# hlesmqh/WS3D

Measured on AMD Instinct MI355X. Metric: KITTI scenes/sec (16384 pts) Stage-1 RPN fwd, 1/2/4/8 GPU; FPS+group HBM GB/s, higher is better.
Workload: dtype f32

## Files before the change

include/ws3d_ops.h:

```cpp
#ifndef WS3D_OPS_H
#define WS3D_OPS_H

#include <stddef.h>
#include <stdint.h>

#ifdef __cplusplus
extern "C" {
#endif

#define WS3D_OK 0
#define WS3D_E_INVALID (-1)
#define WS3D_E_LAUNCH (-2)
#define WS3D_E_WORKSPACE (-3)
#define WS3D_E_UNSUPPORTED (-4)

#if defined(__GNUC__)
#define WS3D_API __attribute__((visibility("default")))
#else
#define WS3D_API
#endif

typedef void *ws3d_stream_t;

#define WS3D_ABI_VERSION 6
// ... 97 lines not shown
WS3D_API int ws3d_pgather_gemm2_compact(int b, int n, int m, long max_rows, int o1, int o2, const float *pmat, int p_stride, const float *xyz,
                               const float *new_xyz, const int32_t *rowc, const int32_t *rowsrc, const int32_t *total, const float *w1x,
                               const float *b1, int relu1, const float *w2t, const float *b2, int relu2, float *out, long limit, ws3d_stream_t stream);
WS3D_API int ws3d_pgather_gemm3_compact(int b, int n, int m, long max_rows, int o1, int o2, int o3, const float *pmat, int p_stride, const float *xyz,
                               const float *new_xyz, const int32_t *rowc, const int32_t *rowsrc, const int32_t *total, const float *w1x,
                               const float *b1, int relu1, const float *w2t, const float *b2, int relu2, const float *w3t, const float *b3,
                               float *out, int out_stride, long limit, ws3d_stream_t stream);
WS3D_API int ws3d_gemm_pool_compact(long max_rows, int k_dim, int o_dim, const float *x_rows, const int32_t *rowc, const int32_t *total,
                           const float *wt, const float *bias, float *out, int out_stride, long limit, ws3d_stream_t stream);
typedef struct ws3d_compact_mlp_args {
    int b, n, m;
    long max_rows;
    int o1, o2, o3;
    const float *pmat;
    int p_stride;
    const float *xyz, *new_xyz;
    const int32_t *rowc, *rowsrc, *total;
    const float *w1x, *b1;
    int relu1;
    const float *w2t, *b2;
    int relu2;
    const float *w3t, *b3;
    float *mid;
    float *out;
    int out_stride;
    long limit;
} ws3d_compact_mlp_args;
WS3D_API int ws3d_compact_mlp_pair(int kind, const ws3d_compact_mlp_args *scale0, const ws3d_compact_mlp_args *scale1, ws3d_stream_t stream);
WS3D_API int ws3d_chain_mlp3_ticket_ints(void);
WS3D_API size_t ws3d_chain_mlp3_blob_floats(int o2);
WS3D_API int ws3d_chain_mlp3_pack(const ws3d_compact_mlp_args *scale, float *blob, ws3d_stream_t stream);
WS3D_API int ws3d_chain_mlp3(const ws3d_compact_mlp_args *scale0, const ws3d_compact_mlp_args *scale1, const float *blob0, const float *blob1,
                             int32_t *ticket, int workgroups, ws3d_stream_t stream);

WS3D_API int ws3d_sa_mlp3_pool_compact(int b, int n, int m, long max_rows, int c1, int c2, int c3, const float *xyz, const float *new_xyz,
                              const float *feat, const int32_t *rowc, const int32_t *rowsrc, const int32_t *total, const float *w1t,
                              const float *b1, const float *w2t, const float *b2, const float *w3t, const float *b3, float *out,
                              int out_stride, long limit, ws3d_stream_t stream);

WS3D_API int ws3d_sa_mlp3_pool_lists(int b, int n, int m, int nsample, int c1, int c2, int c3, const float *xyz, const float *new_xyz,
                            const float *feat, const int32_t *nbr, const float *w1t, const float *b1, const float *w2t, const float *b2,
                            const float *w3t, const float *b3, int relu3, float *out, int out_stride, const int32_t *gate, long gate_limit,
                            ws3d_stream_t stream);

WS3D_API int ws3d_interp_gemm(int b, int n, int m, int c2, int c1, int o_dim, const float *known_feats, const float *unknown_feats,
                     const int32_t *idx, const float *weight, const float *wt, const float *bias, int relu, float *out,
                     ws3d_stream_t stream);

WS3D_API size_t ws3d_conv1x1_wgrad_workspace_bytes(int b, int o, int c, long l);
WS3D_API int ws3d_conv1x1_wgrad(int b, int o, int c, long l, const float *grad_out, const float *x, float *grad_w,
                                void *workspace, size_t workspace_bytes, ws3d_stream_t stream);

WS3D_API size_t ws3d_bn_workspace_bytes(int b, int c, long l);
WS3D_API int ws3d_bn_relu_train_fwd(int b, int c, long l, const float *x, const float *gamma, const float *beta, float eps,
                                    float momentum, int relu, float *running_mean, float *running_var,
                                    int64_t *num_batches_tracked, float *y, float *save_mean, float *save_invstd,
                                    void *workspace, size_t workspace_bytes, ws3d_stream_t stream);
WS3D_API int ws3d_bn_relu_train_bwd(int b, int c, long l, const float *x, const float *dy, const float *gamma,
                                    const float *beta, const float *save_mean, const float *save_invstd, int relu, float *dx,
                                    float *dgamma, float *dbeta, void *workspace, size_t workspace_bytes, ws3d_stream_t stream);

WS3D_API int ws3d_three_interpolate(int b, int c, int m, int n, const float *points, const int32_t *idx,
                           const float *weight, float *out, ws3d_stream_t stream);

WS3D_API int ws3d_three_interpolate_grad(int b, int c, int n, int m, const float *grad_out,
                                const int32_t *idx, const float *weight, float *grad_points,
// ... 188 lines not shown
```

ws3d_amd/_lib.py:

```python
from __future__ import annotations

import ctypes as C
import os

_HERE = os.path.dirname(os.path.abspath(__file__))
DIST_MODE = int(os.environ.get("WS3D_DIST_MODE", "0") or 0)
LIB_PATH = os.environ.get("WS3D_HIP_LIB") or os.path.join(
    _HERE, "libws3d_hip.so" if DIST_MODE == 0 else "libws3d_hip_dm%d.so" % DIST_MODE)

E_INVALID, E_LAUNCH, E_WORKSPACE, E_UNSUPPORTED = -1, -2, -3, -4
ABI_VERSION = 6

_vp = C.c_void_p
_i = C.c_int
_f = C.c_float
_sz = C.c_size_t

class CompactMlpArgs(C.Structure):
    _fields_ = [("b", _i), ("n", _i), ("m", _i), ("max_rows", C.c_long), ("o1", _i), ("o2", _i), ("o3", _i), ("pmat", _vp), ("p_stride", _i),
                ("xyz", _vp), ("new_xyz", _vp), ("rowc", _vp), ("rowsrc", _vp), ("total", _vp), ("w1x", _vp), ("b1", _vp), ("relu1", _i),
                ("w2t", _vp), ("b2", _vp), ("relu2", _i), ("w3t", _vp), ("b3", _vp), ("mid", _vp), ("out", _vp), ("out_stride", _i), ("limit", C.c_long)]


SIGNATURES = {
# ... 53 lines not shown
    "ws3d_topk_sorted_ws": (_i, [_i, _i, _i, _vp, _vp, _vp, _vp, C.c_size_t, _vp]),
    "ws3d_topk_sorted_sigmoid": (_i, [_i, _i, _i, _vp, _vp, _vp, _vp]),
    "ws3d_topk_sorted_sigmoid_ws": (_i, [_i, _i, _i, _vp, _vp, _vp, _vp, C.c_size_t, _vp]),
    "ws3d_three_nn_weights": (_i, [C.c_long, _vp, _vp, _vp]),
    "ws3d_three_nn_w": (_i, [_i, _i, _i, _vp, _vp, _vp, _vp, _vp, _vp, _vp]),
    "ws3d_three_nn_wq": (_i, [_i, _i, _i, _vp, _vp, _vp, _vp, _vp, _vp, _vp, _vp]),
    "ws3d_three_nn_jobs": (_i, [_i, _i, _vp, _vp, _vp, _vp, _vp, _vp, _vp, _vp, _vp]),
    "ws3d_bias_act_inplace": (_i, [_i, _i, C.c_long, _i, _vp, _vp, _vp]),
    "ws3d_rowmax_bias_act": (_i, [_i, _i, C.c_long, _i, _i, _vp, _vp, _vp, _vp]),
    "ws3d_boxes_overlap_bev": (_i, [_i, _vp, _i, _vp, _vp, _vp]),
    "ws3d_boxes_iou_bev": (_i, [_i, _vp, _i, _vp, _vp, _vp]),
    "ws3d_boxes_iou3d_paired": (_i, [_i, _vp, _vp, _vp, _vp, _vp, _vp]),
    "ws3d_nms_mask": (_i, [_i, _vp, _f, _i, _i, _vp, _vp]),
    "ws3d_nms_workspace_bytes": (_sz, [_i]),
    "ws3d_nms": (_i, [_i, _vp, _f, _i, _i, _vp, _sz, _vp, _vp, _vp]),
    "ws3d_nms_batched": (_i, [_i, _i, _vp, _f, _i, _i, _vp, _sz, _vp, _vp, _vp]),
    "ws3d_radius_nms_batched": (_i, [_i, _i, _vp, _f, _i, _vp, _sz, _vp, _vp, _vp]),
    "ws3d_gather_gemm": (_i, [_i, _i, _i, _i, _i, _i, _vp, _vp, _vp, _vp, _vp, _vp, _i, _vp, _vp]),
    "ws3d_gather_gemm2": (_i, [_i, _i, _i, _i, _i, _i, _i, _vp, _vp, _vp, _vp, _vp, _vp, _i, _vp, _vp, _i, _vp, _vp]),
    "ws3d_pgather_gemm2": (_i, [_i, _i, _i, _i, _i, _i, _vp, _i, _vp, _vp, _vp, _vp, _vp, _i, _vp, _vp, _i, _vp, _vp, C.c_long, _vp]),
    "ws3d_pgather_rows": (_i, [_i, _i, _i, _i, _i, _vp, _i, _vp, _vp, _vp, _vp, _vp, _i, _vp, _vp]),
    "ws3d_qinterp_rows": (_i, [_i, _i, _i, _i, _vp, _vp, _vp, _vp, _vp, _i, _vp, _vp, _i, _vp, _vp]),
    "ws3d_compact_pairs": (_i, [C.c_long, _i, _vp, _vp, _vp, _vp, _vp]),
    "ws3d_compact_pairs_count": (_i, [C.c_long, _i, _vp, _vp, _vp]),
    "ws3d_compact_pairs_rows": (_i, [C.c_long, _i, _vp, _vp, _vp, _vp, _vp, _vp, _vp]),
    "ws3d_pgather_gemm2_compact": (_i, [_i, _i, _i, C.c_long, _i, _i, _vp, _i, _vp, _vp, _vp, _vp, _vp, _vp, _vp, _i, _vp, _vp, _i, _vp, C.c_long, _vp]),
    "ws3d_pgather_gemm3_compact": (_i, [_i, _i, _i, C.c_long, _i, _i, _i, _vp, _i, _vp, _vp, _vp, _vp, _vp, _vp, _vp, _i, _vp, _vp, _i, _vp, _vp, _vp, _i, C.c_long, _vp]),
    "ws3d_gemm_pool_compact": (_i, [C.c_long, _i, _i, _vp, _vp, _vp, _vp, _vp, _vp, _i, C.c_long, _vp]),
    "ws3d_compact_mlp_pair": (_i, [_i, C.POINTER(CompactMlpArgs), C.POINTER(CompactMlpArgs), _vp]),
    "ws3d_chain_mlp3_ticket_ints": (_i, []),
    "ws3d_chain_mlp3_blob_floats": (_sz, [_i]),
    "ws3d_chain_mlp3_pack": (_i, [C.POINTER(CompactMlpArgs), _vp, _vp]),
    "ws3d_chain_mlp3": (_i, [C.POINTER(CompactMlpArgs), C.POINTER(CompactMlpArgs), _vp, _vp, _vp, _i, _vp]),
    "ws3d_sa_mlp3_pool_compact": (_i, [_i, _i, _i, C.c_long, _i, _i, _i, _vp, _vp, _vp, _vp, _vp, _vp, _vp, _vp, _vp, _vp, _vp, _vp, _vp, _i, C.c_long, _vp]),
    "ws3d_sa_mlp3_pool_lists": (_i, [_i, _i, _i, _i, _i, _i, _i, _vp, _vp, _vp, _vp, _vp, _vp, _vp, _vp, _vp, _vp, _i, _vp, _i, _vp, C.c_long, _vp]),
    "ws3d_interp_gemm": (_i, [_i, _i, _i, _i, _i, _i, _vp, _vp, _vp, _vp, _vp, _vp, _i, _vp, _vp]),
    "ws3d_gather_boxes_bev": (_i, [_i, _i, _i, _vp, _vp, _vp, _vp, _vp]),
    "ws3d_select_proposals": (_i, [_i, _i, _i, _i, _vp, _vp, _vp, _vp, _f, _vp, _vp, _vp, _vp, _vp]),
    "ws3d_decode_gather_boxes_bev": (_i, [_i, _i, _i, _i, _f, _f, _f, _f, _f, _vp, _vp, _vp, _vp, _vp, _vp]),
    "ws3d_select_proposals_packed": (_i, [_i, _i, _i, _i, _vp, _vp, _vp, _vp, _f, _vp, _vp, _vp, _vp, _vp, _vp]),
    "ws3d_select_proposals_send": (_i, [_i, _i, _i, _i, _vp, _vp, _vp, _vp, _f, _vp, _vp, _vp, _vp, _vp, C.c_long, _vp]),
    "ws3d_split_points_clear": (_i, [C.c_long, _i, _vp, _vp, _vp, _vp, C.c_size_t, _vp]),
    "ws3d_roipool3d": (_i, [_i, _i, _i, _i, _i, _vp, _vp, _vp, _vp, _vp, _vp, _vp]),
    "ws3d_roipool3d_fill": (_i, [_i, _i, _i, _i, _i, _vp, _vp, _vp, _vp, _vp, _vp, _vp]),
    "ws3d_roipool3d_workspace_bytes": (C.c_size_t, [_i, _i]),
    "ws3d_roipool3d_ws": (_i, [_i, _i, _i, _i, _i, _vp, _vp, _vp, _vp, _vp, _vp, _i, _vp, C.c_size_t, _vp]),
    "ws3d_pts_in_boxes3d": (_i, [_i, _i, _vp, _vp, _vp, _vp]),
    "ws3d_instance_clouds": (_i, [_i, _i, _i, _i, _i, _f, _i, _f, _vp, _vp, _vp, _vp, _vp, _vp, _vp, _vp, _vp, _vp]),
    "ws3d_instance_clouds_count": (_i, [_i, _i, _i, _f, _vp, _vp, _vp, _vp, _vp]),
    "ws3d_instance_clouds_emit": (_i, [_i, _i, _i, _i, _f, _i, _f, _vp, _vp, _vp, _vp, _vp, _vp, _vp, _vp, _vp, _vp]),
    "ws3d_click_prepare": (_i, [_i, _i, _i, _i, _vp, _f, _f, _f, _f, _vp, _vp, _vp, _vp, _vp, _vp, _vp]),
    "ws3d_kitti_overlaps": (_i, [_i, _i, _i, C.c_long, _vp, _vp, _vp, _vp, _vp, _vp, _vp]),
    "ws3d_kitti_collect_scores": (_i, [_i, _i, _vp, _vp, _vp, _vp, _vp, _vp, _vp, C.c_double, _vp, _vp, _vp]),
    "ws3d_kitti_count_workspace_bytes": (_sz, [_i, _i]),
    "ws3d_kitti_count": (_i, [_i, _i, _i, _i, _vp, _vp, _vp, _vp, _vp, _vp, _vp, _vp, _vp, _vp, _vp, _vp, _vp, C.c_double, _i, _vp,
                              _sz, _vp, _vp]),
    "ws3d_stage2_embed": (_i, [C.c_long, _i, _vp, _vp, _f] + [_vp] * 10 + [_vp, _vp, _vp]),
    "ws3d_stage2_boxes": (_i, [_i, _i, _i, _f, _f, _f, _f, _vp, _vp, _vp, _vp]),
    "ws3d_stage2_select": (_i, [_i, _i, _f, _f, C.POINTER(_f), _f, _vp, _vp, _vp, _vp, _vp, _vp, _vp, _vp, _vp, _vp]),
    "ws3d_stage2_rcnn_loss": (_i, [_i, _i, _i, _f, _f, _f, _f] + [_vp] * 9 + [_vp]),
    "ws3d_stage2_ioun_loss": (_i, [_i] + [_vp] * 10 + [_vp]),
    "ws3d_rpn_center_labels": (_i, [_i, _i, _i, _i, _f, _f, C.c_double] + [_vp] * 5 + [_vp]),
    "ws3d_rpn_loss_workspace_bytes": (_sz, [_i]),
    "ws3d_rpn_loss": (_i, [_i, _i] + [C.c_double] * 6 + [_vp] * 8 + [_vp, _sz, _vp]),
}

# ... 39 lines not shown
```

ws3d_amd/build.py:

```python
from __future__ import annotations

import argparse
import concurrent.futures as cf
import glob
import os
import shutil
import subprocess
import sys

HERE = os.path.dirname(os.path.abspath(__file__))
CSRC = os.path.join(HERE, "csrc")
OBJ = os.path.join(CSRC, "build")
LIB = os.path.join(HERE, "libws3d_hip.so")
DIST_MODES = (0, 1, 2)


def lib_path(dist_mode: int = 0) -> str:
    return LIB if dist_mode == 0 else os.path.join(HERE, "libws3d_hip_dm%d.so" % dist_mode)
ARCH = "gfx950"
SOURCES = ["core.hip", "fps.hip", "fps_v3.hip", "fps_bucket.hip", "fps_nested.hip", "ballquery_group.hip", "interpolate.hip", "roipool3d.hip", "iou3d.hip", "proposals.hip", "scatter_det.hip", "sa_mlp.hip", "bn_relu.hip", "gemm_pool.hip", "conv_wgrad.hip", "chain_mlp.hip", "rpn_heads.hip", "gemm_rows.hip", "kitti_eval.hip", "instance_clouds.hip", "click.hip", "stage2.hip", "stage2_loss.hip", "rpn_targets.hip"]
CXXFLAGS = ["-O3", "-std=c++17", "-fPIC", "-ffp-contract=off", "-fno-fast-math",
            "-fvisibility=hidden", "-Wall", "-Wno-unused-function"]


def hipcc() -> str:
    for cand in (os.environ.get("HIPCC"), shutil.which("hipcc"), "/opt/rocm/bin/hipcc"):
        if cand and os.path.exists(cand):
            return cand
    raise RuntimeError("hipcc not found (looked at $HIPCC, PATH, /opt/rocm/bin)")


def _deps(src: str):
    return [src, *glob.glob(os.path.join(CSRC, "*.h")), os.path.join(HERE, "..", "include", "ws3d_ops.h"),
            os.path.join(CSRC, "exports.map"), os.path.abspath(__file__)]


def _compile(src: str, force: bool, verbose: bool, dist_mode: int = 0) -> str:
    path = os.path.join(CSRC, src)
    obj = os.path.join(OBJ if dist_mode == 0 else OBJ + "_dm%d" % dist_mode, os.path.splitext(src)[0] + ".o")
    if not force and os.path.exists(obj) and all(
            os.path.getmtime(obj) >= os.path.getmtime(d) for d in _deps(path)):
        return obj
    cmd = [hipcc(), f"--offload-arch={ARCH}", *CXXFLAGS, f"-DWS3D_DIST_MODE={dist_mode}", *os.environ.get("WS3D_EXTRA_DEFS", "").split(), "-c", path, "-o", obj]
    if verbose:
        print(" ".join(cmd), flush=True)
    r = subprocess.run(cmd, capture_output=True, text=True)
    if r.returncode != 0:
        raise RuntimeError(f"hipcc failed for {src}:\n{r.stdout}\n{r.stderr}")
    if verbose and r.stderr.strip():
        print(r.stderr)
    return obj


# ... 43 lines not shown
```

ws3d_amd/compat.py:

```python
from __future__ import annotations

import sys
import types

import os

import torch

from . import _lib
from ._lib import Ws3dError, check


def _dev(*tensors):
    dev = None
    for t in tensors:
        if t is None:
            continue
        if not t.is_cuda:
            raise Ws3dError("ws3d_amd ops need HIP ('cuda') tensors; there is no CPU fallback")
        if not t.is_contiguous():
            raise Ws3dError("ws3d_amd ops need contiguous tensors (the reference asserts the same)")
        if dev is None:
            dev = t.device
        elif t.device != dev:
# ... 578 lines not shown
    O2, O3 = w2t.size(1), w3t.size(1)
    rows = rowc.numel()
    lds = 4 * ((o1 + (O2 + 15) // 16 * 16) * 65 + 2 * 16 * 64)
    if (o1 not in (64, 128) or O2 % 4 or O3 % 128 or lds > min(max_lds, 160 * 1024 - 1024) or pmat.dim() != 2 or pmat.size(0) != B * N or pmat.stride(1) != 1 or
            col0 < 0 or col0 + o1 > pmat.size(1) or tuple(w1x.shape) != (3, o1) or w2t.size(0) != o1 or w3t.size(0) != O2 or not w1x.is_contiguous() or
            not w2t.is_contiguous() or not w3t.is_contiguous() or out2d.dim() != 2 or out2d.stride(1) != 1 or col_offset < 0 or col_offset + O3 > out2d.size(1)):
        return False
    with _on(dev):
        check(_lib.load().ws3d_pgather_gemm3_compact(B, N, M, rows, o1, O2, O3, pmat.data_ptr() + 4 * col0, pmat.stride(0), _p(xyz), _p(new_xyz), _p(rowc),
                                                     _p(rowsrc), _p(total), _p(w1x), _p(b1), int(bool(relu1)), _p(w2t), _p(b2), int(bool(relu2)), _p(w3t), _p(b3),
                                                     out2d.data_ptr() + 4 * col_offset, out2d.stride(0), int(limit), _stream()), "pgather_gemm3_compact")
    return True


def gemm_pool_compact(x_rows, pairs, wt, bias, out2d, col_offset, limit=-1):
    rowc, rowsrc, total = pairs
    dev = _dev(x_rows, rowc, wt, out2d)
    _f32(x_rows, "x_rows"); _f32(wt, "wt"); _f32(out2d, "out2d")
    rows, k = x_rows.shape
    o = wt.size(1)
    if (k % 4 or o % 64 or wt.size(0) != k or rows != rowc.numel() or not x_rows.is_contiguous() or not wt.is_contiguous() or out2d.dim() != 2 or
            out2d.stride(1) != 1 or col_offset < 0 or col_offset + o > out2d.size(1)):
        return False
    with _on(dev):
        check(_lib.load().ws3d_gemm_pool_compact(rows, k, o, _p(x_rows), _p(rowc), _p(total), _p(wt), _p(bias), out2d.data_ptr() + 4 * col_offset,
                                                 out2d.stride(0), int(limit), _stream()), "gemm_pool_compact")
    return True


def compact_mlp_pair(kind, scales, max_lds=160 * 1024, mids=None):
    import ctypes as C
    if len(scales) != 2 or scales[0]["o1"] != scales[1]["o1"]:
        return None if kind == 2 else False
    blocks, keep, outs = [], [], []
    for si, a in enumerate(scales):
        rowc, rowsrc, total = a["pairs"]
        pmat, xyz, new_xyz, w1x, w2t, w3t, out2d, o1, col0, col = a["pmat"], a["xyz"], a["new_xyz"], a["w1x"], a["w2t"], a["w3t"], a["out2d"], a["o1"], a["col0"], a["col_offset"]
        dev = _dev(pmat, xyz, new_xyz, rowc, w1x, w2t, w3t, out2d)
        for t_, nm in ((pmat, "pmat"), (xyz, "xyz"), (new_xyz, "new_xyz"), (w1x, "w1x"), (w2t, "w2t"), (w3t, "w3t"), (out2d, "out2d")):
            _f32(t_, nm)
        B, N, M = xyz.size(0), xyz.size(1), new_xyz.size(1)
        O2, O3 = w2t.size(1), w3t.size(1)
        rows = rowc.numel()
        lds3 = 4 * ((o1 + (O2 + 15) // 16 * 16) * 65 + 2 * 16 * 64)
        ok = (O2 % 4 == 0 and pmat.dim() == 2 and pmat.size(0) == B * N and pmat.stride(1) == 1 and col0 >= 0 and col0 + o1 <= pmat.size(1) and
              tuple(w1x.shape) == (3, o1) and w2t.size(0) == o1 and w3t.size(0) == O2 and w1x.is_contiguous() and w2t.is_contiguous() and w3t.is_contiguous() and
              out2d.dim() == 2 and out2d.stride(1) == 1 and col >= 0 and col + O3 <= out2d.size(1))
        if kind == 3:
            ok = ok and o1 in (64, 128) and O3 % 128 == 0 and lds3 <= min(max_lds, 160 * 1024 - 1024)
        elif kind == 2:
            ok = ok and o1 in (64, 128, 256)
        else:
            ok = ok and O3 % 64 == 0 and mids is not None and tuple(mids[si].shape) == (rows, O2) and mids[si].is_contiguous()
        if not ok:
            return None if kind == 2 else False
        mid = mids[si] if kind == 1 else (torch.empty((rows, O2), dtype=torch.float32, device=dev) if kind == 2 else None)
        outs.append(mid)
        keep.append((pmat, xyz, new_xyz, rowc, rowsrc, total, w1x, w2t, w3t, out2d, mid, a["b1"], a["b2"], a["b3"]))
        blocks.append(_lib.CompactMlpArgs(B, N, M, rows, o1, O2, O3, pmat.data_ptr() + 4 * col0, pmat.stride(0), _p(xyz), _p(new_xyz), _p(rowc), _p(rowsrc),
                                          _p(total), _p(w1x), _p(a["b1"]), int(bool(a["relu1"])), _p(w2t), _p(a["b2"]), int(bool(a["relu2"])), _p(w3t), _p(a["b3"]),
                                          _p(mid), out2d.data_ptr() + 4 * col, out2d.stride(0), -1))
    with _on(dev):
        rc = _lib.load().ws3d_compact_mlp_pair(int(kind), C.byref(blocks[0]), C.byref(blocks[1]), _stream())
    if rc == _lib.E_UNSUPPORTED:
        return None if kind == 2 else False
    check(rc, "compact_mlp_pair")
    return outs if kind == 2 else True


CHAIN_WORKGROUPS = 0
TUNE_KEYS = {"chain_wgs": 0, "mlp2_wgs": 1, "sa1_wgs": 2, "fp_wgs": 3, "pair_wgs": 4, "bq_wide_nw": 5}


def tune(name: str, value: int = -1) -> int:
    rc = _lib.load().ws3d_tune(TUNE_KEYS[name], int(value))
    if rc < 0:
        check(rc, "tune")
    return rc


_CHAIN_BLOBS = {}


def chain_ticket_ints() -> int:
    return int(_lib.load().ws3d_chain_mlp3_ticket_ints())


def _chain_blob(block, tensors, dev):
    import ctypes as C
    key = tuple((t.data_ptr(), t._version) if t is not None else None for t in tensors)
    hit = _CHAIN_BLOBS.get(key)
    if hit is None:
        n = int(_lib.load().ws3d_chain_mlp3_blob_floats(block.o2))
        blob = torch.empty(n, dtype=torch.float32, device=dev)
        with _on(dev):
            check(_lib.load().ws3d_chain_mlp3_pack(C.byref(block), _p(blob), _stream()), "chain_mlp3_pack")
        if torch.cuda.is_current_stream_capturing():
            return blob
        hit = _CHAIN_BLOBS[key] = (blob, tensors)
    return hit[0]


def chain_mlp3(scales, ticket):
    import ctypes as C
# ... 890 lines not shown
```

ws3d_amd/csrc/common.h:

```cpp
#pragma once
#include <hip/hip_runtime.h>
#include <stdint.h>

#include "../../include/ws3d_ops.h"

#define WS3D_WAVE 64

namespace ws3d {

void set_error(const char *fmt, ...);
int check_launch(const char *what);
int raise_lds_cap(const void *fn, size_t bytes, const char *what);
int cu_count();

typedef float floatx16 __attribute__((ext_vector_type(16)));

enum : int { TUNE_CHAIN_WGS = 0, TUNE_MLP2_WGS = 1, TUNE_SA1_WGS = 2, TUNE_FP_WGS = 3, TUNE_PAIR_WGS = 4, TUNE_COUNT = 8 };
extern int g_tune[TUNE_COUNT];

static inline hipStream_t as_stream(ws3d_stream_t s) { return reinterpret_cast<hipStream_t>(s); }

#ifndef WS3D_DIST_MODE
#define WS3D_DIST_MODE 0
#endif
__device__ __forceinline__ float sqdist3(float dx, float dy, float dz) {
#if WS3D_DIST_MODE == 0
    return __builtin_fmaf(dz, dz, __builtin_fmaf(dx, dx, dy * dy));
#elif WS3D_DIST_MODE == 1
    return (dx * dx + dy * dy) + dz * dz;
#else
    return __builtin_fmaf(dz, dz, __builtin_fmaf(dy, dy, dx * dx));
#endif
}

__device__ __forceinline__ float cosf_cr(float a) { return (float)cos((double)a); }
__device__ __forceinline__ float sinf_cr(float a) { return (float)sin((double)a); }
__device__ __forceinline__ float atan2f_cr(float y, float x) { return (float)atan2((double)y, (double)x); }

template <int CTRL>
__device__ __forceinline__ float dpp_f(float v) {
    return __builtin_bit_cast(
        float, __builtin_amdgcn_update_dpp(0, __builtin_bit_cast(int, v), CTRL, 0xF, 0xF, false));
}
enum : int {
    DPP_QUAD_XOR1 = 0xB1,
    DPP_QUAD_XOR2 = 0x4E,
    DPP_ROW_HALF_MIRROR = 0x141,
    DPP_ROW_MIRROR = 0x140,
};

// ... 69 lines not shown
```

ws3d_amd/fastpath.py:

```python
from __future__ import annotations

import contextlib
import contextvars

import torch
import torch.nn as nn

from . import compat as _C
from . import nn_blocks, pn2_ops

FUSED_SA_MLP = True
SA1_FROM_LISTS = True
FUSED_GEMM_POOL = True
FUSED_INTERP_GEMM = True
NESTED_FPS = True
GEOMETRY_AHEAD = True
_AHEAD_OVERRIDE = contextvars.ContextVar("ws3d_geometry_ahead", default=None)


@contextlib.contextmanager
def geometry_ahead(on: bool):
    token = _AHEAD_OVERRIDE.set(bool(on))
    try:
        yield
# ... 2 lines not shown


@contextlib.contextmanager
def compact_only_scales(keys):
    token = _COMPACT_ONLY.set(frozenset(keys))
    try:
        yield
    finally:
        _COMPACT_ONLY.reset(token)


def primed_compact_scales(net, pointcloud: torch.Tensor, margin: float = None):
    margin = PRIMED_MARGIN if margin is None else margin
    keys, per_level = set(), {}
    for row in list_fill(net, pointcloud):
        si = per_level.get(row["level"], 0)
        per_level[row["level"]] = si + 1
        if row["fill"] <= margin * COMPACT_MAX_FILL:
            keys.add((row["level"] - 1, si))
    return frozenset(keys)


def _geometry_ahead_now() -> bool:
    v = _AHEAD_OVERRIDE.get()
    return GEOMETRY_AHEAD if v is None else v
GEOMETRY_IN_CAPTURE = False
PER_POINT_L1 = True
COMPACT_MAX_FILL = 0.55
COMPACT_PAIRS = True
PAIR_DISPATCH = "device"
PRIMED_MARGIN = 0.85
_COMPACT_ONLY = contextvars.ContextVar("ws3d_compact_only_scales", default=frozenset())
CHAIN_MLP = True
PAIRED_SCALES = True
MERGED_THREE_NN = True
FUSED_PROLOGUE = True
MERGED_BINNING = True
PER_POINT_FP = True
FUSED_MLP2_ROWS = True
FUSED_HEADS = True
SPLIT_GEMMS = True
FUSED_GATHER_GEMM2 = True
BIN_INPUT_AHEAD = True
FUSED_QINTERP_GEMM_MIN_ROWS = 30000
FUSED_COMPACT3_MAX_LDS = 64 * 1024
FUSED_GATHER_GEMM = True
GRID_MIN_N = 256
DUAL_SCALE_SEARCH = True
NESTED_CHAIN = True
QUERY_CELL_ORDER = True
PARALLEL_SCALES = True
PARALLEL_HEADS = True


def _row_weights(block):
    w, shift, act = block._folded()
    if act is not None and not isinstance(act, nn.ReLU):
        raise NotImplementedError("fast path supports ReLU / no activation only")
    cache = block.__dict__.get("_row_cache")
    if cache is None or cache[0] is not w:
        cache = (w, w.t().contiguous())
        if not torch.cuda.is_current_stream_capturing():
            block.__dict__["_row_cache"] = cache
    return cache[1], shift, act is not None


def _row_weights_xyz_last(block):
    wt, bias, relu = _row_weights(block)
    cache = block.__dict__.get("_row_cache_xyz_last")
    if cache is None or cache[0] is not wt:
        cache = (wt, torch.cat((wt[3:], wt[:3]), dim=0).contiguous())
        if not torch.cuda.is_current_stream_capturing():
            block.__dict__["_row_cache_xyz_last"] = cache
    return cache[1], bias, relu


def _split_rows(block, wt: torch.Tensor, c2: int):
    cache = block.__dict__.get("_split_cache")
    if cache is None or cache[0] is not wt or cache[1] != c2:
        cache = (wt, c2, wt[:c2].contiguous(), wt[c2:].contiguous())
        if not torch.cuda.is_current_stream_capturing():
            block.__dict__["_split_cache"] = cache
    return cache[2], cache[3]


_SPLIT_GEMM_LIBRARY_WINS = frozenset({(512, 1024, 512)})


def _split_gemm_wins(rows: int, k: int, n: int) -> bool:
    return (rows, k, n) not in _SPLIT_GEMM_LIBRARY_WINS


def _split_gemm(x2d: torch.Tensor, holder, key: str, wt: torch.Tensor, bias=None, relu: bool = False):
    if not SPLIT_GEMMS or x2d.dim() != 2 or not _split_gemm_wins(x2d.size(0), wt.size(0), wt.size(1)):
        return None
    packs = holder.__dict__.get("_gemm_rows_packs")
    ent = None if packs is None else packs.get(key)
    if ent is None or ent[0] is not wt:
        if torch.cuda.is_current_stream_capturing():
            return None
        ent = (wt, _C.gemm_rows_pack(wt))
        holder.__dict__.setdefault("_gemm_rows_packs", {})[key] = ent
    if ent[1] is None:
        return None
    return _C.gemm_rows_split(x2d, ent[1], wt.size(1), bias, relu)


def gemm_rows_packs(model):
    return [ent[1] for m in model.modules() for ent in m.__dict__.get("_gemm_rows_packs", {}).values() if ent[1] is not None]


def _layer(x2d: torch.Tensor, block) -> torch.Tensor:
    wt, bias, relu = _row_weights(block)
    y = _split_gemm(x2d, block, "row", wt, bias, relu)
    if y is not None:
        return y
# ... 387 lines not shown
        rows = g.view(-1, g.size(3))
        if not (FUSED_SA_MLP and rows.size(1) == 4 and len(blocks) == 3 and
                _C.sa_mlp3_pool(rows, grouper.nsample, [_row_weights(b) for b in blocks], out, col)):
            y = rows
            for blk in blocks[:-1]:
                y = _layer(y, blk)
            wt, bias, relu = _row_weights(blocks[-1])
            if not (FUSED_GEMM_POOL and _C.gemm_pool(y, wt, bias, relu, grouper.nsample, out, col)):
                _C.rowmax_rows(_layer(y, blocks[-1]), grouper.nsample, out, col)

    def run_paired() -> bool:
        if not (PAIRED_SCALES and COMPACT_PAIRS and PER_POINT_L1 and len(widths) == 2 and all(isinstance(n_, _PairList) for n_ in nbrs)):
            return False
        blk = [_blocks(m_) for m_ in sa.mlps]
        if any(len(b_) != 3 or b_[0].conv.out_channels > 256 for b_ in blk) or blk[0][0].conv.out_channels != blk[1][0].conv.out_channels:
            return False
        if any(_pair_limit(n_.nbr.numel(), True, (level, si_)) != -1 for si_, n_ in enumerate(nbrs)):
            return False
        if pp[0] is None:
            pp[0] = _per_point_l1(sa, feats, nbrs)
        pmat, offs, w1xs = pp[0]
        scales = []
        for si_ in range(2):
            _w1, b1, r1 = _row_weights_xyz_last(blk[si_][0])
            wt2, b2, r2 = _row_weights(blk[si_][1])
            wt3, b3, r3 = _row_weights(blk[si_][2])
            if not r3:
                return False
            scales.append({"pmat": pmat, "col0": offs[si_], "o1": blk[si_][0].conv.out_channels, "xyz": xyz, "new_xyz": new_xyz, "pairs": nbrs[si_].pairs,
                           "w1x": w1xs[si_], "b1": b1, "relu1": r1, "w2t": wt2, "b2": b2, "relu2": r2, "w3t": wt3, "b3": b3, "out2d": out, "col_offset": cols[si_]})
        if (CHAIN_MLP and zeros is not None and all(sc_["o1"] == 64 and sc_["w2t"].size(1) <= 96 and sc_["w3t"].size(1) == 128 for sc_ in scales)
                and _C.chain_mlp3(scales, zeros.take((_C.chain_ticket_ints(),), torch.int32))):
            return True
        if _C.compact_mlp_pair(3, scales, max_lds=FUSED_COMPACT3_MAX_LDS):
            return True
        mids = _C.compact_mlp_pair(2, scales)
        if mids is None:
            return False
        if not _C.compact_mlp_pair(1, scales, mids=mids):
            for sc_, mid in zip(scales, mids):
                if not _C.gemm_pool_compact(mid, sc_["pairs"], sc_["w3t"], sc_["b3"], out, sc_["col_offset"], limit=-1):
                    raise RuntimeError("ws3d_gemm_pool_compact declined a shape ws3d_pgather_gemm2_compact took")
        return True

    if run_paired():
        pass
    elif geo is not None and geo.aux is not None and PARALLEL_SCALES and len(widths) == 2:
        if PER_POINT_L1 and any(n is not None and len(_blocks(m)) >= 3 for n, m in zip(nbrs, sa.mlps)):
            pp[0] = _per_point_l1(sa, feats, nbrs)
        fork = torch.cuda.Event()
        fork.record(geo.main)
        geo.aux.wait_event(fork)
        with torch.cuda.stream(geo.aux):
            run_scale(1)
            join = torch.cuda.Event()
            join.record(geo.aux)
        run_scale(0)
        geo.main.wait_event(join)
    else:
        for si in range(len(widths)):
            run_scale(si)
    return new_xyz, out.view(B, sa.npoint, -1)


def fp_forward(fp, unknown: torch.Tensor, known: torch.Tensor, unknown_feats, known_feats: torch.Tensor, nn3=None, sorted_unknown=None,
               known_xz=None):
# ... 145 lines not shown
```

Measured before the change: 7009.

## Add persistent stream MLP kernel fusing three layers for SA3/SA4 paired scales

Adds a new persistent HIP kernel that runs layer 1, layer 2 and layer 3 of the per-pair MLP plus max-pool atomics for both scales of the SA3/SA4 modules. Row tiles are kept in LDS, and pre-packed weights are streamed from global memory with MFMA 32x32x2 f32 and one-step prefetch. It is routed ahead of the existing fused compact path when o1 is 128 or 256. The aim is to remove the intermediate activation round-trips and the separate launches. The cost is heavy LDS use per workgroup, which limits occupancy, and a cached weight-blob packing step.

```diff
diff --git a/include/ws3d_ops.h b/include/ws3d_ops.h
--- a/include/ws3d_ops.h
+++ b/include/ws3d_ops.h
@@ -153,6 +153,11 @@
 WS3D_API int ws3d_chain_mlp3_pack(const ws3d_compact_mlp_args *scale, float *blob, ws3d_stream_t stream);
 WS3D_API int ws3d_chain_mlp3(const ws3d_compact_mlp_args *scale0, const ws3d_compact_mlp_args *scale1, const float *blob0, const float *blob1,
                              int32_t *ticket, int workgroups, ws3d_stream_t stream);
+WS3D_API size_t ws3d_stream_mlp_blob_floats(int o1, int o2, int o3);
+WS3D_API int ws3d_stream_mlp_tile_rows(int o1);
+WS3D_API int ws3d_stream_mlp_pack(const ws3d_compact_mlp_args *scale, float *blob, ws3d_stream_t stream);
+WS3D_API int ws3d_stream_mlp(const ws3d_compact_mlp_args *scale0, const ws3d_compact_mlp_args *scale1, const float *blob0, const float *blob1,
+                             int workgroups, ws3d_stream_t stream);
 
 WS3D_API int ws3d_sa_mlp3_pool_compact(int b, int n, int m, long max_rows, int c1, int c2, int c3, const float *xyz, const float *new_xyz,
                               const float *feat, const int32_t *rowc, const int32_t *rowsrc, const int32_t *total, const float *w1t,
diff --git a/ws3d_amd/_lib.py b/ws3d_amd/_lib.py
--- a/ws3d_amd/_lib.py
+++ b/ws3d_amd/_lib.py
@@ -109,6 +109,10 @@
     "ws3d_chain_mlp3_blob_floats": (_sz, [_i]),
     "ws3d_chain_mlp3_pack": (_i, [C.POINTER(CompactMlpArgs), _vp, _vp]),
     "ws3d_chain_mlp3": (_i, [C.POINTER(CompactMlpArgs), C.POINTER(CompactMlpArgs), _vp, _vp, _vp, _i, _vp]),
+    "ws3d_stream_mlp_blob_floats": (_sz, [_i, _i, _i]),
+    "ws3d_stream_mlp_tile_rows": (_i, [_i]),
+    "ws3d_stream_mlp_pack": (_i, [C.POINTER(CompactMlpArgs), _vp, _vp]),
+    "ws3d_stream_mlp": (_i, [C.POINTER(CompactMlpArgs), C.POINTER(CompactMlpArgs), _vp, _vp, _i, _vp]),
     "ws3d_sa_mlp3_pool_compact": (_i, [_i, _i, _i, C.c_long, _i, _i, _i, _vp, _vp, _vp, _vp, _vp, _vp, _vp, _vp, _vp, _vp, _vp, _vp, _vp, _i, C.c_long, _vp]),
     "ws3d_sa_mlp3_pool_lists": (_i, [_i, _i, _i, _i, _i, _i, _i, _vp, _vp, _vp, _vp, _vp, _vp, _vp, _vp, _vp, _vp, _i, _vp, _i, _vp, C.c_long, _vp]),
     "ws3d_interp_gemm": (_i, [_i, _i, _i, _i, _i, _i, _vp, _vp, _vp, _vp, _vp, _vp, _i, _vp, _vp]),
diff --git a/ws3d_amd/build.py b/ws3d_amd/build.py
--- a/ws3d_amd/build.py
+++ b/ws3d_amd/build.py
@@ -18,7 +18,7 @@
 def lib_path(dist_mode: int = 0) -> str:
     return LIB if dist_mode == 0 else os.path.join(HERE, "libws3d_hip_dm%d.so" % dist_mode)
 ARCH = "gfx950"
-SOURCES = ["core.hip", "fps.hip", "fps_v3.hip", "fps_bucket.hip", "fps_nested.hip", "ballquery_group.hip", "interpolate.hip", "roipool3d.hip", "iou3d.hip", "proposals.hip", "scatter_det.hip", "sa_mlp.hip", "bn_relu.hip", "gemm_pool.hip", "conv_wgrad.hip", "chain_mlp.hip", "rpn_heads.hip", "gemm_rows.hip", "kitti_eval.hip", "instance_clouds.hip", "click.hip", "stage2.hip", "stage2_loss.hip", "rpn_targets.hip"]
+SOURCES = ["core.hip", "fps.hip", "fps_v3.hip", "fps_bucket.hip", "fps_nested.hip", "ballquery_group.hip", "interpolate.hip", "roipool3d.hip", "iou3d.hip", "proposals.hip", "scatter_det.hip", "sa_mlp.hip", "bn_relu.hip", "gemm_pool.hip", "conv_wgrad.hip", "chain_mlp.hip", "stream_mlp.hip", "rpn_heads.hip", "gemm_rows.hip", "kitti_eval.hip", "instance_clouds.hip", "click.hip", "stage2.hip", "stage2_loss.hip", "rpn_targets.hip"]
 CXXFLAGS = ["-O3", "-std=c++17", "-fPIC", "-ffp-contract=off", "-fno-fast-math",
             "-fvisibility=hidden", "-Wall", "-Wno-unused-function"]
 
diff --git a/ws3d_amd/compat.py b/ws3d_amd/compat.py
--- a/ws3d_amd/compat.py
+++ b/ws3d_amd/compat.py
@@ -634,6 +634,8 @@
     import ctypes as C
     if len(scales) != 2 or scales[0]["o1"] != scales[1]["o1"]:
         return None if kind == 2 else False
+    if kind == 4:
+        return _stream_mlp_pair(scales)
     blocks, keep, outs = [], [], []
     for si, a in enumerate(scales):
         rowc, rowsrc, total = a["pairs"]
@@ -670,8 +672,66 @@
     return outs if kind == 2 else True
 
 
+_STREAM_BLOBS = {}
+
+
+def stream_mlp_tile_rows(o1: int) -> int:
+    return int(_lib.load().ws3d_stream_mlp_tile_rows(int(o1)))
+
+
+def _stream_blob(block, tensors, dev):
+    import ctypes as C
+    key = (block.o1, block.o2, block.o3) + tuple((t.data_ptr(), t._version) for t in tensors)
+    hit = _STREAM_BLOBS.get(key)
+    if hit is None:
+        n = int(_lib.load().ws3d_stream_mlp_blob_floats(block.o1, block.o2, block.o3))
+        if n == 0:
+            return None
+        blob = torch.empty(n, dtype=torch.float32, device=dev)
+        with _on(dev):
+            check(_lib.load().ws3d_stream_mlp_pack(C.byref(block), _p(blob), _stream()), "stream_mlp_pack")
+        if torch.cuda.is_current_stream_capturing():
+            return blob
+        hit = _STREAM_BLOBS[key] = (blob, tensors)
+    return hit[0]
+
+
+def _stream_mlp_pair(scales):
+    import ctypes as C
+    blocks, keep, blobs = [], [], []
+    for a in scales:
+        rowc, rowsrc, total = a["pairs"]
+        pmat, xyz, new_xyz, w1x, w2t, w3t, out2d, o1, col0, col = a["pmat"], a["xyz"], a["new_xyz"], a["w1x"], a["w2t"], a["w3t"], a["out2d"], a["o1"], a["col0"], a["col_offset"]
+        dev = _dev(pmat, xyz, new_xyz, rowc, w1x, w2t, w3t, out2d)
+        for t_, nm in ((pmat, "pmat"), (xyz, "xyz"), (new_xyz, "new_xyz"), (w1x, "w1x"), (w2t, "w2t"), (w3t, "w3t"), (out2d, "out2d")):
+            _f32(t_, nm)
+        B, N, M = xyz.size(0), xyz.size(1), new_xyz.size(1)
+        O2, O3 = w2t.size(1), w3t.size(1)
+        ok = (o1 in (128, 256) and 0 < O2 <= 384 and O3 % 32 == 0 and pmat.dim() == 2 and pmat.size(0) == B * N and pmat.stride(1) == 1 and pmat.stride(0) % 4 == 0 and
+              col0 >= 0 and col0 % 4 == 0 and col0 + o1 <= pmat.size(1) and tuple(w1x.shape) == (3, o1) and w2t.size(0) == o1 and w3t.size(0) == O2 and
+              w1x.is_contiguous() and w2t.is_contiguous() and w3t.is_contiguous() and out2d.dim() == 2 and out2d.stride(1) == 1 and col >= 0 and
+              col + O3 <= out2d.size(1) and xyz.is_contiguous() and new_xyz.is_contiguous() and rowc.numel() > 0)
+        if not ok:
+            return False
+        keep.append((pmat, xyz, new_xyz, rowc, rowsrc, total, w1x, w2t, w3t, out2d, a["b1"], a["b2"], a["b3"]))
+        blocks.append(_lib.CompactMlpArgs(B, N, M, rowc.numel(), o1, O2, O3, pmat.data_ptr() + 4 * col0, pmat.stride(0), _p(xyz), _p(new_xyz), _p(rowc), _p(rowsrc),
+                                          _p(total), _p(w1x), _p(a["b1"]), int(bool(a["relu1"])), _p(w2t), _p(a["b2"]), int(bool(a["relu2"])), _p(w3t), _p(a["b3"]),
+                                          None, out2d.data_ptr() + 4 * col, out2d.stride(0), int(a.get("limit", -1))))
+        if pmat.data_ptr() % 16:
+            return False
+        blobs.append(_stream_blob(blocks[-1], (w2t, w3t), dev))
+        if blobs[-1] is None:
+            return False
+    with _on(dev):
+        rc = _lib.load().ws3d_stream_mlp(C.byref(blocks[0]), C.byref(blocks[1]), _p(blobs[0]), _p(blobs[1]), 0, _stream())
+    if rc == _lib.E_UNSUPPORTED:
+        return False
+    check(rc, "stream_mlp")
+    return True
+
+
 CHAIN_WORKGROUPS = 0
-TUNE_KEYS = {"chain_wgs": 0, "mlp2_wgs": 1, "sa1_wgs": 2, "fp_wgs": 3, "pair_wgs": 4, "bq_wide_nw": 5}
+TUNE_KEYS = {"chain_wgs": 0, "mlp2_wgs": 1, "sa1_wgs": 2, "fp_wgs": 3, "pair_wgs": 4, "bq_wide_nw": 5, "stream_wgs": 6}
 
 
 def tune(name: str, value: int = -1) -> int:
diff --git a/ws3d_amd/csrc/common.h b/ws3d_amd/csrc/common.h
--- a/ws3d_amd/csrc/common.h
+++ b/ws3d_amd/csrc/common.h
@@ -15,7 +15,7 @@
 
 typedef float floatx16 __attribute__((ext_vector_type(16)));
 
-enum : int { TUNE_CHAIN_WGS = 0, TUNE_MLP2_WGS = 1, TUNE_SA1_WGS = 2, TUNE_FP_WGS = 3, TUNE_PAIR_WGS = 4, TUNE_COUNT = 8 };
+enum : int { TUNE_CHAIN_WGS = 0, TUNE_MLP2_WGS = 1, TUNE_SA1_WGS = 2, TUNE_FP_WGS = 3, TUNE_PAIR_WGS = 4, TUNE_STREAM_WGS = 6, TUNE_COUNT = 8 };
 extern int g_tune[TUNE_COUNT];
 
 static inline hipStream_t as_stream(ws3d_stream_t s) { return reinterpret_cast<hipStream_t>(s); }
diff --git a/ws3d_amd/csrc/stream_mlp.hip b/ws3d_amd/csrc/stream_mlp.hip
--- /dev/null
+++ b/ws3d_amd/csrc/stream_mlp.hip
@@ -0,0 +1,284 @@
+#include <algorithm>
+
+#include "common.h"
+#include "compact_pool.h"
+
+#ifndef WS3D_STREAM_AHEAD
+#define WS3D_STREAM_AHEAD 1
+#endif
+#ifndef WS3D_STREAM_SA3_RH
+#define WS3D_STREAM_SA3_RH 3
+#define WS3D_STREAM_SA3_WAVES 8
+#define WS3D_STREAM_SA3_PER_CU 1
+#endif
+#ifndef WS3D_STREAM_SA4_RH
+#define WS3D_STREAM_SA4_RH 1
+#define WS3D_STREAM_SA4_WAVES 8
+#define WS3D_STREAM_SA4_PER_CU 2
+#endif
+
+namespace ws3d {
+
+struct StreamScale {
+    const float *pmat, *xyz, *new_xyz;
+    const int32_t *rowc, *rowsrc, *total;
+    const float *w1x, *b1, *b2, *b3, *blob;
+    float *out;
+    long limit;
+    int o2, o3, n, m, p_stride, relu1, relu2, out_stride, j2;
+};
+
+struct StreamPair { StreamScale s[2]; };
+
+__host__ __device__ constexpr size_t stream_blob_floats(int o1, int j2, int o3) { return (size_t)o1 * 32 * j2 + (size_t)32 * j2 * o3; }
+
+__global__ __launch_bounds__(256) void stream_pack_kernel(int o1, int o2, int o3, const float *__restrict__ w2t, const float *__restrict__ w3t,
+                                                          float *__restrict__ blob) {
+    const int o2p = (o2 + 31) / 32 * 32;
+    const long n2 = (long)o1 * o2p, n3 = (long)o2p * o3;
+    float *w3l = blob + n2;
+    for (long i = (long)blockIdx.x * 256 + threadIdx.x; i < n2 + n3; i += (long)gridDim.x * 256) {
+        if (i < n2) {
+            const int k = (int)(i / o2p), o = (int)(i - (long)k * o2p);
+            const int s = k >> 1, h = k & 1;
+            blob[(((long)(s >> 2) * 2 + h) * o2p + o) * 4 + (s & 3)] = o < o2 ? w2t[(long)k * o2 + o] : 0.f;
+        } else {
+            const long i3 = i - n2;
+            const int k = (int)(i3 / o3), o = (int)(i3 - (long)k * o3);
+            const int s = k >> 1, h = k & 1;
+            w3l[(((long)(s >> 2) * 2 + h) * o3 + o) * 4 + (s & 3)] = k < o2 ? w3t[(long)k * o3 + o] : 0.f;
+        }
+    }
+}
+
+__device__ __forceinline__ float f4_at(const float4 &v, int e) { return e == 0 ? v.x : e == 1 ? v.y : e == 2 ? v.z : v.w; }
+
+template <int RH, bool TRANSPOSED>
+__device__ __forceinline__ void stream_layer(floatx16 (&acc)[RH], const float4 *__restrict__ wl, long wstride, const float4 *xl, int kb) {
+    constexpr int ROWS = 32 * RH;
+    float4 ca = wl[0], cb = wl[wstride];
+#if WS3D_STREAM_AHEAD == 2
+    float4 ma = wl[(long)min(2, kb - 2) * wstride], mb = wl[(long)(min(2, kb - 2) + 1) * wstride];
+#endif
+#pragma unroll 1
+    for (int blk = 0; blk < kb; blk += 2) {
+        const int nx = min(blk + 2 * WS3D_STREAM_AHEAD, kb - 2);
+        const float4 na = wl[(long)nx * wstride], nb = wl[(long)(nx + 1) * wstride];
+        __builtin_amdgcn_sched_barrier(0);
+#pragma unroll
+        for (int u = 0; u < 2; ++u) {
+            const float4 wv = u ? cb : ca;
+            float4 x[RH];
+#pragma unroll
+            for (int r = 0; r < RH; ++r) x[r] = xl[(blk + u) * 2 * ROWS + 32 * r];
+#pragma unroll
+            for (int e = 0; e < 4; ++e)
+#pragma unroll
+                for (int r = 0; r < RH; ++r)
+                    acc[r] = TRANSPOSED ? __builtin_amdgcn_mfma_f32_32x32x2f32(f4_at(wv, e), f4_at(x[r], e), acc[r], 0, 0, 0)
+                                        : __builtin_amdgcn_mfma_f32_32x32x2f32(f4_at(x[r], e), f4_at(wv, e), acc[r], 0, 0, 0);
+        }
+        __builtin_amdgcn_sched_barrier(0);
+#if WS3D_STREAM_AHEAD == 2
+        ca = ma; cb = mb; ma = na; mb = nb;
+#else
+        ca = na; cb = nb;
+#endif
+    }
+}
+
+template <int RH>
+__device__ __forceinline__ void stream_store_act(const floatx16 &acc, const float *__restrict__ bias, int relu, int ch0, int o_valid, float *act, int row, int h,
+                                                 const float *__restrict__ safe) {
+    constexpr int ROWS = 32 * RH;
+#pragma unroll
+    for (int q = 0; q < 4; ++q) {
+        float y[4];
+#pragma unroll
+        for (int i = 0; i < 4; ++i) {
+            const int ch = ch0 + 8 * q + 4 * h + i;
+            const bool in = ch < o_valid;
+            const float bl = *(bias ? bias + min(ch, o_valid - 1) : safe);
+            const float bv = bias ? bl : 0.f;
+            float v = acc[4 * q + i] + bv;
+            if (relu) v = v < 0.f ? 0.f : v;
+            y[i] = in ? v : 0.f;
+        }
+        float *dst = act + ((long)((ch0 / 8 + q) * 2) * ROWS + row) * 4 + 2 * h;
+        *reinterpret_cast<float2 *>(dst) = make_float2(y[0], y[2]);
+        *reinterpret_cast<float2 *>(dst + ROWS * 4) = make_float2(y[1], y[3]);
+    }
+}
+
+template <int NB1, int RH, int WAVES>
+__device__ __forceinline__ void stream_tile(const StreamScale *base, long off, float *act1, float *act2, const long tile, const long T, const int wave, const int h, const int c) {
+    constexpr int O1 = 64 * NB1, ROWS = 32 * RH;
+    const long row0 = tile * ROWS;
+#define WS3D_STREAM_BLOCK()                 \
+    asm volatile("" : "+s"(off));           \
+    const StreamScale &a = *reinterpret_cast<const StreamScale *>(reinterpret_cast<const char *>(base) + off)
+    {
+    WS3D_STREAM_BLOCK();
+    for (int unit = wave; unit < (O1 / 32) * RH; unit += WAVES) {
+        const int j = unit / RH, r = unit - j * RH;
+        const long t = min(row0 + 32 * r + c, T - 1);
+        const int cm = a.rowc[t];
+        const int src = a.rowsrc[t];
+        const size_t pnt = (size_t)(cm / a.m) * a.n + (size_t)src;
+        const float *prow = a.pmat + pnt * a.p_stride + 32 * j + 4 * h;
+        floatx16 acc;
+#pragma unroll
+        for (int q = 0; q < 4; ++q) {
+            const float4 v = *reinterpret_cast<const float4 *>(prow + 8 * q);
+            acc[4 * q + 0] = v.x; acc[4 * q + 1] = v.y; acc[4 * q + 2] = v.z; acc[4 * q + 3] = v.w;
+        }
+        const float *pr = a.xyz + pnt * 3, *cr = a.new_xyz + (size_t)cm * 3;
+        const float dx = pr[0] - cr[0], dy = pr[1] - cr[1], dz = pr[2] - cr[2];
+        const float bxy = h ? dy : dx, bz = h ? 0.f : dz;
+        const float wa0 = a.w1x[h * O1 + 32 * j + c], wa1 = h ? 0.f : a.w1x[2 * O1 + 32 * j + c];
+        acc = __builtin_amdgcn_mfma_f32_32x32x2f32(wa0, bxy, acc, 0, 0, 0);
+        acc = __builtin_amdgcn_mfma_f32_32x32x2f32(wa1, bz, acc, 0, 0, 0);
+        stream_store_act<RH>(acc, a.b1, a.relu1, 32 * j, O1, act1, 32 * r + c, h, a.w1x);
+    }
+    }
+    lds_barrier();
+    {
+    WS3D_STREAM_BLOCK();
+    const int o2p = 32 * a.j2;
+    const float4 *blob4 = reinterpret_cast<const float4 *>(a.blob);
+    for (int jo = wave; jo < a.j2; jo += WAVES) {
+        floatx16 acc[RH];
+#pragma unroll
+        for (int r = 0; r < RH; ++r)
+#pragma unroll
+            for (int i = 0; i < 16; ++i) acc[r][i] = 0.f;
+        stream_layer<RH, true>(acc, blob4 + (long)h * o2p + 32 * jo + c, 2L * o2p, reinterpret_cast<const float4 *>(act1) + h * ROWS + c, O1 / 8);
+#pragma unroll
+        for (int r = 0; r < RH; ++r) stream_store_act<RH>(acc[r], a.b2, a.relu2, 32 * jo, a.o2, act2, 32 * r + c, h, a.w1x);
+    }
+    }
+    lds_barrier();
+    {
+    WS3D_STREAM_BLOCK();
+    const int o2p = 32 * a.j2;
+    const float4 *blob4 = reinterpret_cast<const float4 *>(a.blob);
+    const float4 *w3l = blob4 + (long)O1 / 4 * o2p;
+    int cen[RH][16];
+#pragma unroll
+    for (int r = 0; r < RH; ++r) {
+        const int first = (int)row0 + 32 * r + 16 * h, last = (int)T - 1;
+#pragma unroll
+        for (int i = 0; i < 16; ++i) {
+            const int v = a.rowc[min(first + i, last)];
+            cen[r][i] = first + i <= last ? v : -1;
+        }
+    }
+    for (int jc = wave; jc < a.o3 / 32; jc += WAVES) {
+        floatx16 acc[RH];
+#pragma unroll
+        for (int r = 0; r < RH; ++r)
+#pragma unroll
+            for (int i = 0; i < 16; ++i) acc[r][i] = 0.f;
+        stream_layer<RH, false>(acc, w3l + (long)h * a.o3 + 32 * jc + c, 2L * a.o3, reinterpret_cast<const float4 *>(act2) + h * ROWS + c, 4 * a.j2);
+        const int col = 32 * jc + c;
+        const float bv = a.b3 ? a.b3[col] : 0.f;
+#pragma unroll
+        for (int r = 0; r < RH; ++r) {
+            if (row0 + 32 * r >= T) continue;
+#pragma unroll
+            for (int i = 0; i < 16; ++i) asm volatile("" : "+v"(cen[r][i]));
+            compact_pool_atomic(acc[r], bv, cen[r], a.out + col, a.out_stride);
+            __builtin_amdgcn_sched_barrier(0);
+        }
+    }
+    }
+#undef WS3D_STREAM_BLOCK
+}
+
+template <int NB1, int RH, int WAVES>
+__global__ __launch_bounds__(64 * WAVES) void stream_mlp_pair_kernel(const StreamPair p) {
+    extern __shared__ __attribute__((aligned(16))) float stream_smem[];
+    constexpr int O1 = 64 * NB1, ROWS = 32 * RH;
+    const int tid = threadIdx.x, wave = __builtin_amdgcn_readfirstlane(tid >> 6), lane = tid & 63, h = lane >> 5, c = lane & 31;
+    long T0 = *p.s[0].total, T1 = *p.s[1].total;
+    if (p.s[0].limit >= 0 && T0 > p.s[0].limit) T0 = 0;
+    if (p.s[1].limit >= 0 && T1 > p.s[1].limit) T1 = 0;
+    const long tiles0 = (T0 + ROWS - 1) / ROWS, tiles = tiles0 + (T1 + ROWS - 1) / ROWS;
+    float *act1 = stream_smem, *act2 = stream_smem + O1 * ROWS;
+    for (long tile = blockIdx.x; tile < tiles; tile += gridDim.x) {
+        const bool second = tile >= tiles0;
+        long off = second ? (long)sizeof(StreamScale) : 0;
+        stream_tile<NB1, RH, WAVES>(&p.s[0], off, act1, act2, second ? tile - tiles0 : tile, second ? T1 : T0, wave, h, c);
+    }
+}
+
+constexpr int STREAM_SA3_RH = WS3D_STREAM_SA3_RH, STREAM_SA3_WAVES = WS3D_STREAM_SA3_WAVES, STREAM_SA4_RH = WS3D_STREAM_SA4_RH, STREAM_SA4_WAVES = WS3D_STREAM_SA4_WAVES;
+constexpr int STREAM_SA3_PER_CU = WS3D_STREAM_SA3_PER_CU, STREAM_SA4_PER_CU = WS3D_STREAM_SA4_PER_CU;
+constexpr int stream_max_o2(int o1) { return std::min(384, (160 * 1024 / (128 * (o1 == 128 ? STREAM_SA3_RH : STREAM_SA4_RH)) - o1) / 32 * 32); }
+
+}
+
+static bool stream_widths_ok(int o1, int o2, int o3) { return (o1 == 128 || o1 == 256) && o2 > 0 && o2 <= ws3d::stream_max_o2(o1) && o3 > 0 && !(o3 & 31); }
+
+extern "C" size_t ws3d_stream_mlp_blob_floats(int o1, int o2, int o3) {
+    return stream_widths_ok(o1, o2, o3) ? ws3d::stream_blob_floats(o1, (o2 + 31) / 32, o3) : 0;
+}
+
+extern "C" int ws3d_stream_mlp_tile_rows(int o1) { return o1 == 128 ? 32 * ws3d::STREAM_SA3_RH : o1 == 256 ? 32 * ws3d::STREAM_SA4_RH : 0; }
+
+extern "C" int ws3d_stream_mlp_pack(const ws3d_compact_mlp_args *scale, float *blob, ws3d_stream_t stream) {
+    using namespace ws3d;
+    if (!scale || !blob || (reinterpret_cast<uintptr_t>(blob) & 15)) { set_error("ws3d_stream_mlp_pack: invalid argument"); return WS3D_E_INVALID; }
+    if (!stream_widths_ok(scale->o1, scale->o2, scale->o3) || !scale->w2t || !scale->w3t) {
+        set_error("ws3d_stream_mlp_pack: block not covered (o1=%d o2=%d o3=%d; o1 in {128, 256}, o2 <= %d, o3 %% 32)", scale->o1, scale->o2, scale->o3, stream_max_o2(scale->o1));
+        return WS3D_E_UNSUPPORTED;
+    }
+    const size_t n = stream_blob_floats(scale->o1, (scale->o2 + 31) / 32, scale->o3);
+    hipLaunchKernelGGL(stream_pack_kernel, dim3((unsigned)std::min<size_t>(256, (n + 255) / 256)), dim3(256), 0, as_stream(stream), scale->o1, scale->o2, scale->o3,
+                       scale->w2t, scale->w3t, blob);
+    return check_launch("ws3d_stream_mlp_pack");
+}
+
+extern "C" int ws3d_stream_mlp(const ws3d_compact_mlp_args *p0, const ws3d_compact_mlp_args *p1, const float *blob0, const float *blob1, int workgroups,
+                               ws3d_stream_t stream) {
+    using namespace ws3d;
+    if (!p0 || !p1 || !blob0 || !blob1 || ((reinterpret_cast<uintptr_t>(blob0) | reinterpret_cast<uintptr_t>(blob1)) & 15)) {
+        set_error("ws3d_stream_mlp: invalid argument");
+        return WS3D_E_INVALID;
+    }
+    const ws3d_compact_mlp_args *ps[2] = {p0, p1};
+    const float *blobs[2] = {blob0, blob1};
+    StreamPair a;
+    const int rows = ws3d_stream_mlp_tile_rows(p0->o1);
+    long max_tiles = 0;
+    int j2max = 0;
+    for (int i = 0; i < 2; ++i) {
+        const ws3d_compact_mlp_args &q = *ps[i];
+        const bool ok = rows > 0 && q.o1 == p0->o1 && stream_widths_ok(q.o1, q.o2, q.o3) && q.max_rows > 0 && q.max_rows <= 0x3fffffffL && q.b > 0 && q.n > 0 && q.m > 0 &&
+                        q.p_stride >= q.o1 && !(q.p_stride & 3) && !(reinterpret_cast<uintptr_t>(q.pmat) & 15) && q.pmat && q.xyz && q.new_xyz && q.rowc && q.rowsrc &&
+                        q.total && q.w1x && q.out && q.out_stride >= q.o3;
+        if (!ok) {
+            set_error("ws3d_stream_mlp: block %d not covered (rows<=%ld o1=%d o2=%d o3=%d p_stride=%d; equal o1 in {128, 256}, o2 <= %d, o3 %% 32, 16-byte aligned P rows)", i,
+                      q.max_rows, q.o1, q.o2, q.o3, q.p_stride, stream_max_o2(q.o1));
+            return WS3D_E_UNSUPPORTED;
+        }
+        a.s[i] = StreamScale{q.pmat, q.xyz, q.new_xyz, q.rowc, q.rowsrc, q.total, q.w1x, q.b1, q.b2, q.b3, blobs[i], q.out, q.limit,
+                           q.o2, q.o3, q.n, q.m, q.p_stride, q.relu1, q.relu2, q.out_stride, (q.o2 + 31) / 32};
+        max_tiles += (q.max_rows + rows - 1) / rows;
+        j2max = std::max(j2max, a.s[i].j2);
+    }
+    const size_t lds = sizeof(float) * (size_t)(p0->o1 + 32 * j2max) * rows;
+    if (lds > 160 * 1024) { set_error("ws3d_stream_mlp: %zu B of LDS", lds); return WS3D_E_UNSUPPORTED; }
+    long wgs = workgroups > 0 ? workgroups : (g_tune[TUNE_STREAM_WGS] > 0 ? g_tune[TUNE_STREAM_WGS] : (long)cu_count() * (p0->o1 == 128 ? STREAM_SA3_PER_CU : STREAM_SA4_PER_CU));
+    wgs = std::max(1L, std::min(wgs, max_tiles));
+    hipStream_t st = as_stream(stream);
+#define WS3D_STREAM_GO(NB1, RH, WAVES)                                                                                                \
+    do {                                                                                                                              \
+        if (int rc = raise_lds_cap((const void *)stream_mlp_pair_kernel<NB1, RH, WAVES>, lds, "ws3d_stream_mlp")) return rc;          \
+        hipLaunchKernelGGL((stream_mlp_pair_kernel<NB1, RH, WAVES>), dim3((unsigned)wgs), dim3(64 * WAVES), lds, st, a);     \
+    } while (0)
+    if (p0->o1 == 128) WS3D_STREAM_GO(2, STREAM_SA3_RH, STREAM_SA3_WAVES);
+    else WS3D_STREAM_GO(4, STREAM_SA4_RH, STREAM_SA4_WAVES);
+#undef WS3D_STREAM_GO
+    return check_launch("ws3d_stream_mlp");
+}
diff --git a/ws3d_amd/fastpath.py b/ws3d_amd/fastpath.py
--- a/ws3d_amd/fastpath.py
+++ b/ws3d_amd/fastpath.py
@@ -58,6 +58,7 @@
 PRIMED_MARGIN = 0.85
 _COMPACT_ONLY = contextvars.ContextVar("ws3d_compact_only_scales", default=frozenset())
 CHAIN_MLP = True
+STREAM_MLP = True
 PAIRED_SCALES = True
 MERGED_THREE_NN = True
 FUSED_PROLOGUE = True
@@ -108,6 +109,13 @@
         if not torch.cuda.is_current_stream_capturing():
             block.__dict__["_split_cache"] = cache
     return cache[2], cache[3]
+
+
+_STREAM_MLP_PAIR_WINS = frozenset()
+
+
+def _stream_mlp_takes(scales) -> bool:
+    return STREAM_MLP and scales[0]["o1"] in (128, 256) and scales[0]["o1"] not in _STREAM_MLP_PAIR_WINS
 
 
 _SPLIT_GEMM_LIBRARY_WINS = frozenset({(512, 1024, 512)})
@@ -561,6 +569,8 @@
         if (CHAIN_MLP and zeros is not None and all(sc_["o1"] == 64 and sc_["w2t"].size(1) <= 96 and sc_["w3t"].size(1) == 128 for sc_ in scales)
                 and _C.chain_mlp3(scales, zeros.take((_C.chain_ticket_ints(),), torch.int32))):
             return True
+        if _stream_mlp_takes(scales) and _C.compact_mlp_pair(4, scales):
+            return True
         if _C.compact_mlp_pair(3, scales, max_lds=FUSED_COMPACT3_MAX_LDS):
             return True
         mids = _C.compact_mlp_pair(2, scales)
```

New measurement: 7041, median of 4. About the same (+0.5%).
